# staghado/vit.cpp

Measured on AMD Instinct MI355X. Metric: images/sec ViT-B/16 224^2 bs=256 per GPU (forward, synthetic, HBM-resident inputs), higher is better.
Workload: dtype bf16; 1 GPU; vit_base_patch16_224 bf16, batch=256/GPU, 224x224x3 f32 HWC in HBM, random-init f16 file; graph=whole reference graph (every token row of every layer), global_batch=256, parallelism=single GPU

## Files before the change

include/vitx.h:

```cpp
#ifndef VITX_H
#define VITX_H

#include <stddef.h>
#include <stdint.h>

#ifdef __cplusplus
extern "C" {
#endif

typedef struct vitx_model vitx_model;
typedef struct vitx_ctx vitx_ctx;

enum vitx_status {
    VITX_OK = 0,
    VITX_ERR_IO = 1,
    VITX_ERR_FORMAT = 2,
    VITX_ERR_ARG = 3,
    VITX_ERR_HIP = 4,
    VITX_ERR_UNSUPPORTED = 5,
    VITX_ERR_NOMEM = 6
};

enum vitx_dtype { VITX_F16 = 0, VITX_BF16 = 1, VITX_MXFP8 = 2 };

// ... 190 lines not shown
int vitx_feat_enable(vitx_ctx *c, int flags, uint64_t layer_mask);
int vitx_feat_floats(const vitx_ctx *c);
int vitx_feat_images(const vitx_ctx *c);
int vitx_feat_read(vitx_ctx *c, float *out, size_t n_floats);
const void *vitx_feat_device(const vitx_ctx *c);
int vitx_op_features(const void *d_x, long row_stride, long img_stride, const void *d_w, const void *d_b,
                     void *d_cls, void *d_mean, void *d_tokens, long out_img_stride,
                     int n_img, int N, int D, float eps, int l2, void *stream);
int vitx_op_features_ex(const void *d_x, long row_stride, long img_stride, const void *d_w, const void *d_b,
                        void *d_cls, void *d_mean, void *d_tokens, long out_img_stride,
                        int n_img, int N, int first, int D, float eps, int l2, void *d_z, int dtype, void *stream);
int vitx_op_patch_embed_rect(int dtype, const void *d_img , const void *d_w, const void *d_bias, const void *d_pos, const void *d_cls,
                             const void *d_reg, int R, int n_img, int img_h, int img_w, int P, int Cin, int D, void *d_X);
int vitx_op_patch_embed(int dtype, const void *d_img, const void *d_w, const void *d_bias, const void *d_pos, const void *d_cls, const void *d_reg, int R,
                        void *d_X, int n_img, int S, int P, int Cin, int D, void *stream);
int vitx_op_attention_pool(const void *d_x, long row_stride, long img_stride, const void *d_ln_w, const void *d_ln_b, float eps, const void *d_u, void *d_M,
                           void *d_p , int n_img, int N, int D, int H, void *stream);

enum vitx_zs_kind { VITX_ZS_SOFTMAX = 0, VITX_ZS_SIGMOID = 1 };
int vitx_zeroshot_set(vitx_ctx *c, const float *bank , int K, int E, int kind, float scale, float bias);
int vitx_zeroshot_classes(const vitx_ctx *c);
int vitx_zeroshot_images(const vitx_ctx *c);
int vitx_zeroshot_read(vitx_ctx *c, float *probs , float *logits , size_t n_floats_each);
const void *vitx_zeroshot_device(const vitx_ctx *c);
int vitx_zeroshot_max_classes(int E);
int vitx_op_zeroshot(int dtype, const void *d_z, long z_stride, const void *d_bank ,
                     void *d_a_scratch, void *d_acc_scratch, void *d_probs, void *d_logits, int n, int K, int E, int kind, float scale, float bias, void *stream);

enum vitx_nn_source { VITX_NN_LOGITS = 0, VITX_NN_EMBED = 1 };
int vitx_nn_width(const vitx_ctx *c, int source);
// ... 98 lines not shown
```

vit.cpp_amd/binding.py:

```python
from __future__ import annotations

import ctypes as C
import os
import subprocess
from typing import List, Optional, Tuple

import numpy as np

from .ggml_file import (ACT_TANH as ACT_GELU_TANH, ACT_ERF as ACT_GELU_ERF, ACT_QUICK as ACT_QUICK_GELU,
                        ZS_SOFTMAX, ZS_SIGMOID, POOL_CLS, POOL_CLS_MEAN, POOL_MAP,
                        PP_REF_BICUBIC, PP_REF_BILINEAR, PP_PIL_BILINEAR, PP_PIL_BICUBIC, PP_STRETCH, PP_SHORTEST_EDGE)

_HERE = os.path.dirname(os.path.abspath(__file__))
LIB_PATH = os.environ.get("VITX_LIB") or os.path.join(_HERE, "libvitx.so")

F16, BF16, MXFP8 = 0, 1, 2
LN_TEST_KEY = 0x7e570000
BICUBIC, BILINEAR = 0, 1
EPI_BIAS, EPI_BIAS_GELU, EPI_BIAS_RESID, EPI_BIAS_F32, EPI_PATCH, EPI_BIAS_HILO = 0, 1, 2, 3, 4, 5
EPI_BIAS_GELU_ERF, EPI_BIAS_QGELU = 6, 7
ERR_IO, ERR_FORMAT, ERR_ARG, ERR_HIP, ERR_UNSUPPORTED, ERR_NOMEM = 1, 2, 3, 4, 5, 6
GEMM_AUTO, GEMM_PP, GEMM_AUTO_SPLIT = 0, 1, 2
ATTN_AUTO, ATTN_SINGLE, ATTN_FLOW, ATTN_PERSIST, ATTN_STREAM = 0, 1, 3, 4, 5
ATTN_ROLLOUT = 1
# ... 21 lines not shown
    "vitx_model_num_registers", "vitx_model_head_pool", "vitx_ctx_registers", "vitx_op_features_ex", "vitx_op_patch_embed",
    "vitx_model_activation", "vitx_model_has_pre_norm", "vitx_op_layernorm_f32",
    "vitx_model_preproc", "vitx_model_has_preproc", "vitx_preproc_at_size", "vitx_preprocess_ex", "vitx_preprocess_ex_device", "vitx_preprocess_ex_device_supports",
    "vitx_model_num_prefix", "vitx_model_pool_query", "vitx_op_attention_pool",
    "vitx_zeroshot_set", "vitx_zeroshot_classes", "vitx_zeroshot_images", "vitx_zeroshot_read", "vitx_zeroshot_device", "vitx_zeroshot_max_classes", "vitx_op_zeroshot",
    "vitx_nn_width", "vitx_nn_set", "vitx_nn_rows", "vitx_nn_k", "vitx_nn_labels", "vitx_nn_images", "vitx_nn_read", "vitx_nn_device", "vitx_nn_scratch_bytes",
    "vitx_op_nn_select", "vitx_op_nn_finish", "vitx_op_nn_state_bytes", "vitx_op_nn",
    "vitx_dense_set", "vitx_dense_classes", "vitx_dense_shape", "vitx_dense_images", "vitx_dense_read", "vitx_dense_device", "vitx_dense_scratch_bytes",
    "vitx_op_dense_labels", "vitx_dense_labels_host", "vitx_op_dense",
    "vitx_depth_set", "vitx_depth_bins", "vitx_depth_shape", "vitx_depth_images", "vitx_depth_read", "vitx_depth_device", "vitx_depth_scratch_bytes",
    "vitx_op_depth_fine", "vitx_op_depth_resize", "vitx_depth_host", "vitx_op_depth", "vitx_op_depth_rows",
    "vitx_model_kind", "vitx_model_text_info", "vitx_model_text_zs", "vitx_text_create", "vitx_text_free", "vitx_text_embed", "vitx_text_embed_device", "vitx_text_shares_weights", "vitx_text_check_ids",
    "vitx_op_text_embed", "vitx_op_text_pool", "vitx_op_attention_text", "vitx_op_attention_generic",
    "vitx_model_rope", "vitx_model_rope_table", "vitx_op_rope",
    "vitx_model_glu", "vitx_op_swiglu",
    "vitx_ctx_create_rect", "vitx_ctx_img_shape", "vitx_ctx_grid", "vitx_op_patch_embed_rect",
    "vitx_rect_shape", "vitx_preprocess_rect", "vitx_preprocess_rect_device", "vitx_preprocess_rect_device_supports",
    "vitx_pack_create", "vitx_pack_free", "vitx_pack_shares_weights", "vitx_pack_check", "vitx_pack_distinct_grids", "vitx_pack_forward", "vitx_pack_forward_device",
    "vitx_pack_feat_enable", "vitx_pack_feat_read", "vitx_pack_scratch_bytes", "vitx_pack_launches", "vitx_op_attention_packed", "vitx_op_attention_packed_tables", "vitx_op_rope_packed",
]


class HParams(C.Structure):
    _fields_ = [("hidden_size", C.c_int32), ("num_hidden_layers", C.c_int32), ("num_attention_heads", C.c_int32), ("num_classes", C.c_int32),
                ("patch_size", C.c_int32), ("img_size", C.c_int32), ("ftype", C.c_int32), ("eps", C.c_float)]


class CtxOptions(C.Structure):
    _fields_ = [("struct_size", C.c_int32), ("streams", C.c_int32), ("graph", C.c_int32), ("quant_on_host", C.c_int32), ("q4_fused_rows", C.c_int32),
                ("split_first", C.c_int32), ("no_ln_fusion", C.c_int32), ("ln_test", C.c_int32), ("f16_fast_attention", C.c_int32), ("last_layer_all_rows", C.c_int32),
                ("img_size", C.c_int32), ("pos_interp", C.c_int32)]
# ... 215 lines not shown
            L.vitx_op_attention_text.argtypes = [ip, vp, vp, ip, ip, ip, ip, ip, vp]
            L.vitx_op_attention_generic.argtypes = [ip, vp, vp, ip, ip, ip, ip, vp]
        if hasattr(L, "vitx_op_rope"):
            L.vitx_model_rope.argtypes = [vp, C.POINTER(ip), C.POINTER(C.c_float)]
            L.vitx_model_rope_table.argtypes = [vp, ip, ip, C.POINTER(C.c_float), C.POINTER(C.c_float)]
            L.vitx_op_rope.argtypes = [ip, vp, C.c_long, vp, vp, ip, ip, ip, ip, ip, vp]
        if hasattr(L, "vitx_op_swiglu"):
            L.vitx_model_glu.argtypes = [vp, C.POINTER(ip), C.POINTER(ip)]
            L.vitx_op_swiglu.argtypes = [ip, vp, C.c_long, vp, C.c_long, C.c_long, ip, vp]
        if hasattr(L, "vitx_ctx_create_rect"):
            pp = C.POINTER(Preproc)
            L.vitx_ctx_create_rect.argtypes = [vp, ip, ip, ip, C.POINTER(CtxOptions), ip, ip, C.POINTER(vp)]
            L.vitx_ctx_img_shape.argtypes = [vp, C.POINTER(ip), C.POINTER(ip)]
            L.vitx_ctx_grid.argtypes = [vp, C.POINTER(ip), C.POINTER(ip)]
            L.vitx_op_patch_embed_rect.argtypes = [ip, vp, vp, vp, vp, vp, vp, ip, ip, ip, ip, ip, ip, ip, vp]
            L.vitx_rect_shape.argtypes = [ip, ip, ip, ip, ip, C.POINTER(ip), C.POINTER(ip)]
            L.vitx_preprocess_rect.argtypes = [pp, C.POINTER(C.c_uint8), ip, ip, ip, ip, C.POINTER(C.c_float)]
            L.vitx_preprocess_rect_device.argtypes = [pp, vp, ip, ip, ip, ip, ip, vp, vp]
            L.vitx_preprocess_rect_device_supports.argtypes = [pp, ip, ip, ip, ip]
        if hasattr(L, "vitx_pack_create"):
            i32p, fp = C.POINTER(C.c_int32), C.POINTER(C.c_float)
            L.vitx_pack_create.argtypes = [vp, ip, ip, ip, ip, C.POINTER(PackOptions), C.POINTER(vp)]
            L.vitx_pack_free.argtypes = [vp]
            L.vitx_pack_shares_weights.argtypes = [vp]
            L.vitx_pack_check.argtypes = [vp, i32p, ip, ip, ip, i32p]
            L.vitx_pack_distinct_grids.argtypes = [vp, i32p, ip]
            L.vitx_pack_forward.argtypes = [vp, fp, i32p, ip, fp, fp]
            L.vitx_pack_forward_device.argtypes = [vp, vp, i32p, ip, vp, vp, vp]
            L.vitx_pack_feat_enable.argtypes = [vp, ip]
            L.vitx_pack_feat_read.argtypes = [vp, fp, fp]
# ... 872 lines not shown
                   n_img: int, N: int, first: int, D: int, eps: float = 1e-6, l2: bool = False, d_z: int = 0, dtype: int = F16, stream: int = 0) -> None:
    check(lib().vitx_op_features_ex(d_x, row_stride, img_stride, d_w, d_b, d_cls or None, d_mean or None, d_tokens or None, out_img_stride,
                                    n_img, N, first, D, eps, int(l2), d_z or None, dtype, stream or None), "vitx_op_features_ex")


def op_patch_embed(dtype: int, d_img: int, d_w: int, d_bias: int, d_pos: int, d_cls: int, d_reg: int, R: int, d_X: int, n_img: int, S: int, P: int,
                   Cin: int, D: int, stream: int = 0) -> None:
    check(lib().vitx_op_patch_embed(dtype, d_img, d_w, d_bias, d_pos, d_cls or None, d_reg or None, R, d_X, n_img, S, P, Cin, D, stream or None), "vitx_op_patch_embed")


def op_patch_embed_rect(dtype: int, d_img: int, d_w: int, d_bias: int, d_pos: int, d_cls: int, d_reg: int, R: int, d_X: int, n_img: int, img_h: int, img_w: int,
                        P: int, Cin: int, D: int) -> None:
    check(lib().vitx_op_patch_embed_rect(dtype, d_img, d_w, d_bias, d_pos, d_cls or None, d_reg or None, R, n_img, img_h, img_w, P, Cin, D, d_X), "vitx_op_patch_embed_rect")


def op_attention_pool(d_x: int, row_stride: int, img_stride: int, d_ln_w: int, d_ln_b: int, eps: float, d_u: int, d_M: int, d_p: int,
                      n_img: int, N: int, D: int, H: int, stream: int = 0) -> None:
    check(lib().vitx_op_attention_pool(d_x, row_stride, img_stride, d_ln_w, d_ln_b, eps, d_u, d_M, d_p or None, n_img, N, D, H, stream or None), "vitx_op_attention_pool")


def op_rope(dtype: int, d_qkv: int, d_cos: int, d_sin: int, n_img: int, N: int, prefix: int, D: int, H: int, lo_off: int = 0, stream: int = 0) -> None:
    check(lib().vitx_op_rope(dtype, d_qkv, lo_off, d_cos, d_sin, n_img, N, prefix, D, H, stream), "vitx_op_rope")


def op_swiglu(dtype: int, d_in: int, ld_in: int, d_out: int, ld_out: int, rows: int, F: int, stream: int = 0) -> None:
    check(lib().vitx_op_swiglu(dtype, d_in, ld_in, d_out, ld_out, rows, F, stream or None), "vitx_op_swiglu")


def op_text_embed(table_f16: bool, d_tok: int, d_pos: int, d_ids: int, d_x: int, n: int, T: int, D: int, stream: int = 0) -> None:
    check(lib().vitx_op_text_embed(1 if table_f16 else 0, d_tok, d_pos, d_ids, d_x, n, T, D, stream), "vitx_op_text_embed")
# ... 204 lines not shown
```

vit.cpp_amd/csrc/kernels.h:

```cpp
#pragma once
#include <hip/hip_runtime.h>
#include <stdint.h>

#include <type_traits>

#include "../../include/vitx.h"

namespace vitx {

enum { DT_F16 = 0, DT_BF16 = 1 };

enum {
    EPI_BIAS = 0,
    EPI_BIAS_GELU = 1,
    EPI_BIAS_RESID = 2,
    EPI_BIAS_F32 = 3,
    EPI_PATCH = 4,
    EPI_BIAS_HILO = 5,
    EPI_BIAS_GELU_ERF = 6,
    EPI_BIAS_QGELU = 7
};
constexpr int EPI_COUNT = 8;
constexpr __host__ __device__ bool epi_is_act(int epi) { return epi == EPI_BIAS_GELU || epi == EPI_BIAS_GELU_ERF || epi == EPI_BIAS_QGELU; }
constexpr __host__ __device__ int epi_act(int epi) { return epi == EPI_BIAS_GELU_ERF ? 1 : epi == EPI_BIAS_QGELU ? 2 : 0; }
// ... 61 lines not shown
    int attn_grid = 0;
};
const Tuning *tuning_for_device(int device);

hipError_t launch_gemm(const Tuning &t, int dtype, int epi, const GemmArgs &a, hipStream_t stream);
bool gemm_ln_fusable(const Tuning &t, const GemmArgs &a);
bool gemm_fix_capable(const Tuning &t, const GemmArgs &a);
int gemm_ln_grid(int n_cu, int M, int N);
hipError_t launch_layernorm_fixup(int dtype, const float *x, const float *w, const float *b, void *y, int M, int D, float eps, const unsigned *todo, unsigned epoch, hipStream_t stream);
int gemm_ring_cfg(const Tuning &t, const GemmArgs &a);
int gemm_tile_m();
int gemm_tile_n();

hipError_t launch_patch_embed(int dtype, const float *img, const void *w_perm, const float *bias, const float *pos, const float *cls, const float *reg, int n_reg,
                              float *X, int n_img, int img_h, int img_w, int P, int Cin, int D, int n_pad, int k_pad, hipStream_t stream);
void patch_embed_permute_k(const uint16_t *w, uint16_t *w_perm, int N, int Cin, int P, int k_pad);
hipError_t launch_layernorm(int dtype, const float *x, long ldx, const float *w, const float *b, void *y, long ldy, int M, int D, float eps, hipStream_t stream, int group = 1, long gstride = 0);
hipError_t launch_layernorm_f32(const float *x, const float *w, const float *b, float *y, int M, int D, float eps, hipStream_t stream);
hipError_t launch_attention(const Tuning &t, int dtype, const void *qkv, void *out, int n_img, int N, int D, int H, hipStream_t stream);
hipError_t launch_attention_stream(int dtype, bool precise, const void *qkv, void *out, int n_img, int N, int D, int H, long lo_off, hipStream_t stream);
bool attention_stream_supports(int n_img, int N, int D, int H);
hipError_t launch_split_hilo(int dtype, const float *x, void *hi, void *lo, size_t n, hipStream_t stream);
hipError_t launch_attention_cls(int dtype, const void *qkv, long lo_off, void *out, const float *x, float *xc, int n_img, int N, int D, int H, hipStream_t stream);
bool attention_cls_supports(int N, int D, int H);
constexpr int kAttnMeanMaxTokens = 1024;
bool attention_map_supports(int N, int D, int H);
bool attention_mean_supports(int N, int D, int H);
hipError_t launch_attention_cls_map(int dtype, const void *qkv, long lo_off, float *out, long img_stride, int n_img, int N, int D, int H, hipStream_t stream);
hipError_t launch_attention_head_mean(int dtype, const void *qkv, long lo_off, float *out, int n_img, int N, int D, int H, bool half_identity, hipStream_t stream);
hipError_t launch_rollout_step(float *a, const float *r, int n_img, int N, hipStream_t stream);
// ... 98 lines not shown
```

vit.cpp_amd/csrc/ops.cpp:

```cpp
#include <cmath>
#include <initializer_list>

#include "context.h"
#include "preproc_resample.h"
#include "dense_resample.h"

static int op_rc(const char *name, hipError_t e, int invalid = VITX_ERR_HIP) {
    if (e == hipSuccess) return VITX_OK;
    set_error("%s: %s", name, hipGetErrorString(e));
    return e == hipErrorInvalidValue ? invalid : VITX_ERR_HIP;
}
static bool lo_plane_ok(const char *name, int dtype, long lo_off, long hi_elems) {
    if (!lo_off || (dtype == VITX_F16 && lo_off >= hi_elems && lo_off % 8 == 0)) return true;
    set_error("%s: a lo plane needs VITX_F16 and lo_off %ld a multiple of 8 elements, at least n_img * N * 3 * D = %ld", name, lo_off, hi_elems);
    return false;
}

extern "C" {

int vitx_op_layernorm(int dtype, const void *x, const void *w, const void *b, void *y, int M, int D, float eps, void *stream) {
    if (!x || !w || !b || !y || M <= 0) return VITX_ERR_ARG;
    return op_rc("vitx_op_layernorm", launch_layernorm(dtype, (const float *)x, D, (const float *)w, (const float *)b, y, D, M, D, eps, (hipStream_t)stream), VITX_ERR_UNSUPPORTED);
}
int vitx_op_layernorm_f32(const void *x, const void *w, const void *b, void *y, int M, int D, float eps, void *stream) {
// ... 229 lines not shown
        if ((uintptr_t)p % 16) { set_error("%s: pointers must be 16-byte aligned", name); return VITX_ERR_ARG; }
    if (row_stride % 4 || img_stride % 4 || out_img_stride % 4) { set_error("%s: strides must be multiples of 4 floats", name); return VITX_ERR_ARG; }
    if (!layernorm_supports(D)) { set_error("%s: hidden size %d has no LayerNorm instantiation", name, D); return VITX_ERR_UNSUPPORTED; }
    return op_rc(name, launch_features((const float *)d_x, row_stride, img_stride, (const float *)d_w, (const float *)d_b, (float *)d_cls, (float *)d_mean, (float *)d_tokens,
                                       out_img_stride, n_img, N, D, eps, l2 != 0, (hipStream_t)stream, first, d_z, dtype));
}
int vitx_op_features(const void *d_x, long row_stride, long img_stride, const void *d_w, const void *d_b, void *d_cls, void *d_mean, void *d_tokens, long out_img_stride,
                     int n_img, int N, int D, float eps, int l2, void *stream) {
    return op_features("vitx_op_features", false, d_x, row_stride, img_stride, d_w, d_b, d_cls, d_mean, d_tokens, out_img_stride, n_img, N, 1, D, eps, l2, nullptr, VITX_F16, stream);
}
int vitx_op_features_ex(const void *d_x, long row_stride, long img_stride, const void *d_w, const void *d_b, void *d_cls, void *d_mean, void *d_tokens, long out_img_stride,
                        int n_img, int N, int first, int D, float eps, int l2, void *d_z, int dtype, void *stream) {
    return op_features("vitx_op_features_ex", true, d_x, row_stride, img_stride, d_w, d_b, d_cls, d_mean, d_tokens, out_img_stride, n_img, N, first, D, eps, l2, d_z, dtype, stream);
}
static int op_patch_embed(const char *name, int dtype, const void *d_img, const void *d_w, const void *d_bias, const void *d_pos, const void *d_cls, const void *d_reg, int R, void *d_X,
                          int n_img, int img_h, int img_w, int P, int Cin, int D, void *stream) {
    if (!d_img || !d_w || !d_bias || !d_pos || (!d_cls && R != 0) || !d_X || R < 0 || (R > 0 && !d_reg) || n_img <= 0 || img_h <= 0 || img_w <= 0 || P <= 0 || img_h % P || img_w % P ||
        Cin <= 0 || D <= 0 || D % 4 || (dtype != VITX_F16 && dtype != VITX_BF16)) { set_error("%s: invalid argument", name); return VITX_ERR_ARG; }
    if (!tuning_for_device(-1)) { set_error("%s: kernel bring-up failed", name); return VITX_ERR_HIP; }
    const int K = Cin * P * P, k_pad = round_up(K, 64), n_pad = round_up(D, gemm_tile_n());
    std::vector<float> wf((size_t)D * K);
    HIP_TRY(hipMemcpy(wf.data(), d_w, wf.size() * 4, hipMemcpyDeviceToHost));
    const std::vector<uint16_t> hp = operand_matrix_host(dtype, wf.data(), nullptr, D, K, n_pad, k_pad, P, Cin);
    void *w_perm = nullptr; float *bias = nullptr;
    HIP_TRY(hipMalloc(&w_perm, hp.size() * 2));
    const DevMem w_own(w_perm);
    if (hipMalloc((void **)&bias, (size_t)n_pad * 4) != hipSuccess) return VITX_ERR_NOMEM;
    const DevMem bias_own(bias);
    hipStream_t st = (hipStream_t)stream;
    hipError_t e = hipMemcpy(w_perm, hp.data(), hp.size() * 2, hipMemcpyHostToDevice);
    if (e == hipSuccess) e = hipMemset(bias, 0, (size_t)n_pad * 4);
    if (e == hipSuccess) e = hipMemcpy(bias, d_bias, (size_t)D * 4, hipMemcpyDeviceToDevice);
    if (e == hipSuccess) e = launch_patch_embed(dtype, (const float *)d_img, w_perm, bias, (const float *)d_pos, (const float *)d_cls, (const float *)d_reg, R,
                                                (float *)d_X, n_img, img_h, img_w, P, Cin, D, n_pad, k_pad, st);
    if (e == hipSuccess) e = hipStreamSynchronize(st);
    return op_rc(name, e, VITX_ERR_UNSUPPORTED);
}
int vitx_op_patch_embed(int dtype, const void *d_img, const void *d_w, const void *d_bias, const void *d_pos, const void *d_cls, const void *d_reg, int R, void *d_X,
                        int n_img, int S, int P, int Cin, int D, void *stream) {
    return op_patch_embed("vitx_op_patch_embed", dtype, d_img, d_w, d_bias, d_pos, d_cls, d_reg, R, d_X, n_img, S, S, P, Cin, D, stream);
}
int vitx_op_patch_embed_rect(int dtype, const void *d_img, const void *d_w, const void *d_bias, const void *d_pos, const void *d_cls, const void *d_reg, int R,
                             int n_img, int img_h, int img_w, int P, int Cin, int D, void *d_X) {
    return op_patch_embed("vitx_op_patch_embed_rect", dtype, d_img, d_w, d_bias, d_pos, d_cls, d_reg, R, d_X, n_img, img_h, img_w, P, Cin, D, nullptr);
}
int vitx_op_attention_pool(const void *d_x, long row_stride, long img_stride, const void *d_ln_w, const void *d_ln_b, float eps, const void *d_u, void *d_M, void *d_p,
                           int n_img, int N, int D, int H, void *stream) {
    if (!d_x || !d_ln_w || !d_ln_b || !d_u || !d_M || n_img <= 0 || N <= 0 || D <= 0 || H <= 0 || H > kPoolMaxHeads) { set_error("vitx_op_attention_pool: invalid argument (1 <= H <= %d)", kPoolMaxHeads); return VITX_ERR_ARG; }
    for (const void *p : {d_x, d_ln_w, d_ln_b, d_u, (const void *)d_M, (const void *)d_p})
        if ((uintptr_t)p % 16) { set_error("vitx_op_attention_pool: pointers must be 16-byte aligned"); return VITX_ERR_ARG; }
    if (row_stride % 4 || img_stride % 4) { set_error("vitx_op_attention_pool: strides must be multiples of 4 floats"); return VITX_ERR_ARG; }
    if (!layernorm_supports(D)) { set_error("vitx_op_attention_pool: hidden size %d has no LayerNorm instantiation", D); return VITX_ERR_UNSUPPORTED; }
    return op_rc("vitx_op_attention_pool", launch_attention_pool((const float *)d_x, row_stride, img_stride, (const float *)d_ln_w, (const float *)d_ln_b, eps, (const float *)d_u,
                                                                 (float *)d_M, nullptr, DT_F16, (float *)d_p, n_img, N, D, H, (hipStream_t)stream), VITX_ERR_UNSUPPORTED);
}
int vitx_op_attention_map(int dtype, const void *d_qkv, long lo_off, void *d_cls, void *d_mean, int n_img, int N, int D, int H, void *stream) {
    if (!d_qkv || (!d_cls && !d_mean) || n_img <= 0 || N <= 0 || D <= 0 || H <= 0 || (dtype != VITX_F16 && dtype != VITX_BF16)) { set_error("vitx_op_attention_map: invalid argument"); return VITX_ERR_ARG; }
    if (!lo_plane_ok("vitx_op_attention_map", dtype, lo_off, (long)n_img * N * 3 * D)) return VITX_ERR_ARG;
    if (!attention_map_supports(N, D, H)) { set_error("vitx_op_attention_map: head_dim must be a multiple of 8 up to 128 (D %d, H %d)", D, H); return VITX_ERR_UNSUPPORTED; }
// ... 235 lines not shown
```

vit.cpp_amd/csrc/patch_embed.hip:

```cpp
#include "device_common.h"
#include "kernels.h"
#include "epilogue16.h"

namespace vitx {

namespace pe {
constexpr int BM = 128, BN = 128, BK = 64;
constexpr int TILE = BM * BK * 2, STAGE = 2 * TILE, LDS_BYTES = 2 * STAGE;
}

template <typename T>
__global__ __launch_bounds__(256) void patch_embed_kernel(GemmArgs g, const float *__restrict__ img, const float *__restrict__ cls, const float *__restrict__ reg, int IH, int IW , int P, int Cin, int gw ) {
    using namespace pe;
    extern __shared__ __attribute__((aligned(16))) char smem[];
    typedef typename Elem<T>::v8 v8;
    const int tid = threadIdx.x, lane = tid & 63;
    const int wave = __builtin_amdgcn_readfirstlane(tid >> 6);
    const int l15 = lane & 15, g4 = lane >> 4;

    const int nwg = gridDim.x, bid = blockIdx.x;
    const int q8 = nwg >> 3, r8 = nwg & 7, xcd = bid & 7;
    const int tile = (xcd < r8 ? xcd * (q8 + 1) : r8 * (q8 + 1) + (xcd - r8) * q8) + (bid >> 3);
    const int ntn = g.N_pad / BN;
    const int m0 = (tile / ntn) * BM, n0 = (tile % ntn) * BN;

    const T *W = (const T *)g.W;
    int woff[4];
#pragma unroll
    for (int i = 0; i < 4; ++i) { int row, slot; swz_inv(i * 256 + tid, row, slot); woff[i] = (n0 + row) * g.ldw + slot * 8; }
    auto stage_w = [&](int buf, int k0) {
        char *base = smem + buf * STAGE + TILE + wave * 1024;
#pragma unroll
        for (int i = 0; i < 4; ++i) __builtin_amdgcn_global_load_lds(GPTR(W + woff[i] + k0), LPTR(base + i * 4096), 16, 0, 0);
    };
    const int a_row = tid >> 1, a_h = tid & 1;
    const int K = Cin * P * P, PC = P * Cin, tpi = g.tpi;
    const int m = m0 + a_row;
    const bool row_ok = m < g.M_real;
    const float *prow;
    {
        const int b = m / tpi, t = m - b * tpi, py = t / gw, px = t - py * gw;
        prow = img + (((size_t)b * IH + (size_t)py * P) * IW + (size_t)px * P) * Cin;
    }
    const bool fast = (PC & 15) == 0;
    f32x4 areg[2][4];
    auto load_a = [&](int kt) {
#pragma unroll
        for (int q = 0; q < 2; ++q) {
            const int k0 = kt * BK + (a_h * 2 + q) * 16;
            if (fast) {
                const int ky = k0 / PC, r0 = k0 - ky * PC;
                const f32x4 *src = (const f32x4 *)(prow + (size_t)ky * IW * Cin + r0);
                const bool ok = row_ok && k0 < K;
#pragma unroll
                for (int e = 0; e < 4; ++e) areg[q][e] = ok ? src[e] : f32x4{0.0f, 0.0f, 0.0f, 0.0f};
            } else {
#pragma unroll
                for (int e = 0; e < 16; ++e) {
                    const int k = k0 + e, ky = k / PC, r = k - ky * PC;
                    areg[q][e >> 2][e & 3] = (row_ok && k < K) ? prow[(size_t)ky * IW * Cin + r] : 0.0f;
                }
            }
        }
    };
    auto write_a = [&](int buf) {
        char *at = smem + buf * STAGE;
#pragma unroll
        for (int q = 0; q < 2; ++q)
#pragma unroll
            for (int hh = 0; hh < 2; ++hh) {
                const f32x4 lo = areg[q][2 * hh], hi = areg[q][2 * hh + 1];
                const typename Pair<T>::v2 p0 = round_pair<T>(lo[0], lo[1]), p1 = round_pair<T>(lo[2], lo[3]), p2 = round_pair<T>(hi[0], hi[1]), p3 = round_pair<T>(hi[2], hi[3]);
                *(v8 *)(at + swz_byte(a_row, (a_h * 2 + q) * 2 + hh)) = v8{p0[0], p0[1], p1[0], p1[1], p2[0], p2[1], p3[0], p3[1]};
            }
    };

    const int wm = wave >> 1, wn = wave & 1;
    f32x4 acc[4][4];
#pragma unroll
    for (int t = 0; t < 4; ++t)
#pragma unroll
        for (int u = 0; u < 4; ++u) acc[t][u] = f32x4{0.0f, 0.0f, 0.0f, 0.0f};
    int a_rd[4][2], w_rd[4][2];
#pragma unroll
    for (int t = 0; t < 4; ++t)
#pragma unroll
        for (int k2 = 0; k2 < 2; ++k2) {
            a_rd[t][k2] = swz_byte(wm * 64 + t * 16 + l15, k2 * 4 + g4);
            w_rd[t][k2] = TILE + swz_byte(wn * 64 + t * 16 + l15, k2 * 4 + g4);
        }

    const int nk = g.K / BK;
    stage_w(0, 0);
    load_a(0); write_a(0);
    asm volatile("s_waitcnt vmcnt(0)" ::: "memory");
    __syncthreads();
    for (int kt = 0; kt < nk; ++kt) {
        const int cur = kt & 1;
        if (kt + 1 < nk) { stage_w(cur ^ 1, (kt + 1) * BK); load_a(kt + 1); }
        const char *sb = smem + cur * STAGE;
#pragma unroll
        for (int k2 = 0; k2 < 2; ++k2) {
            v8 af[4], wf[4];
#pragma unroll
            for (int t = 0; t < 4; ++t) { af[t] = *(const v8 *)(sb + a_rd[t][k2]); wf[t] = *(const v8 *)(sb + w_rd[t][k2]); }
#pragma unroll
            for (int t = 0; t < 4; ++t)
#pragma unroll
                for (int u = 0; u < 4; ++u) acc[t][u] = Elem<T>::mfma16(wf[u], af[t], acc[t][u]);
        }
        if (kt + 1 < nk) write_a(cur ^ 1);
        asm volatile("s_waitcnt vmcnt(0)" ::: "memory");
        __syncthreads();
    }
    const bool full = (m0 + BM <= g.M_real) && (n0 + BN <= g.N);
    const int row0 = m0 + wm * 64 + l15, col0 = n0 + wn * 64 + 4 * g4;
    if (full) epilogue16<T, EPI_PATCH, 4, 4, true>(g, acc, row0, col0);
    else epilogue16<T, EPI_PATCH, 4, 4, false>(g, acc, row0, col0);
    if (g.prefix == 0) return;
#pragma unroll
    for (int t = 0; t < 4; ++t) {
        const int row = row0 + t * 16;
        if (row >= g.M_real || row % tpi) continue;
        float *o = (float *)g.out + ((size_t)row + (size_t)(row / tpi) * g.prefix) * g.ldo;
#pragma unroll
        for (int u = 0; u < 4; ++u)
#pragma unroll
            for (int e = 0; e < 4; ++e) { const int c = col0 + u * 16 + e; if (c < g.N) o[c] = cls[c] + g.pos[c]; }
// ... 5 lines not shown
#pragma unroll
                for (int e = 0; e < 4; ++e) { const int c = col0 + u * 16 + e; if (c < g.N) orow[c] = src[c]; }
        }
    }
}

void patch_embed_permute_k(const uint16_t *w, uint16_t *w_perm, int N, int Cin, int P, int k_pad) {
    const int K = Cin * P * P;
    for (int n = 0; n < N; ++n)
        for (int c = 0; c < Cin; ++c)
            for (int y = 0; y < P; ++y)
                for (int x = 0; x < P; ++x) w_perm[(size_t)n * k_pad + (y * P + x) * Cin + c] = w[(size_t)n * k_pad + c * P * P + y * P + x];
    (void)K;
}

hipError_t prepare_patch_embed() {
    hipError_t e = hipFuncSetAttribute((const void *)patch_embed_kernel<_Float16>, hipFuncAttributeMaxDynamicSharedMemorySize, pe::LDS_BYTES);
    if (e != hipSuccess) return e;
    return hipFuncSetAttribute((const void *)patch_embed_kernel<__bf16>, hipFuncAttributeMaxDynamicSharedMemorySize, pe::LDS_BYTES);
}

hipError_t launch_patch_embed(int dtype, const float *img, const void *w_perm, const float *bias, const float *pos, const float *cls, const float *reg, int n_reg,
                              float *X, int n_img, int img_h, int img_w, int P, int Cin, int D, int n_pad, int k_pad, hipStream_t stream) {
    if (n_img <= 0 || P <= 0 || img_h <= 0 || img_w <= 0 || img_h % P || img_w % P || n_pad % pe::BN || k_pad % pe::BK || k_pad < Cin * P * P || D % 4 || n_reg < 0 || (n_reg > 0 && (!reg || !cls))) return hipErrorInvalidValue;
    const int gh = img_h / P, gw = img_w / P, tpi = gh * gw;
    if ((long)n_img * tpi > 0x7fffff00l) return hipErrorInvalidValue;
    GemmArgs g{};
    g.W = w_perm; g.bias = bias; g.out = X; g.pos = pos;
    g.M_real = n_img * tpi; g.M = (g.M_real + pe::BM - 1) / pe::BM * pe::BM; g.N = D; g.N_pad = n_pad; g.K = k_pad; g.ldw = k_pad; g.ldo = D; g.tpi = tpi; g.prefix = cls ? 1 + n_reg : 0;
    const int grid = (g.M / pe::BM) * (n_pad / pe::BN);
    if (dtype == DT_F16) hipLaunchKernelGGL(patch_embed_kernel<_Float16>, dim3(grid), dim3(256), pe::LDS_BYTES, stream, g, img, cls, reg, img_h, img_w, P, Cin, gw);
    else hipLaunchKernelGGL(patch_embed_kernel<__bf16>, dim3(grid), dim3(256), pe::LDS_BYTES, stream, g, img, cls, reg, img_h, img_w, P, Cin, gw);
    return hipGetLastError();
}

}
```

Measured before the change: 27010 images/s.

## Add wide-tile triple-buffered patch-embed kernel with direct LDS DMA for weights

Rewrites the patch-embedding GEMM kernel so the weight operand uses three LDS buffers filled by inline global_load_lds DMA. Image loads are issued two k-steps ahead with partial vmcnt waits in place of a full drain every iteration. It also adds a 256-column tile variant with 512 threads, chosen automatically when the grid still covers all CUs, and compile-time FAST/slow im2col paths using 32-bit offsets. The goal is to hide global-load latency and improve weight reuse in the patch embed, at the cost of more template instances, more registers and tighter offset-range limits.

```diff
diff --git a/include/vitx.h b/include/vitx.h
--- a/include/vitx.h
+++ b/include/vitx.h
@@ -228,6 +228,8 @@
                              const void *d_reg, int R, int n_img, int img_h, int img_w, int P, int Cin, int D, void *d_X);
 int vitx_op_patch_embed(int dtype, const void *d_img, const void *d_w, const void *d_bias, const void *d_pos, const void *d_cls, const void *d_reg, int R,
                         void *d_X, int n_img, int S, int P, int Cin, int D, void *stream);
+int vitx_op_patch_embed_ex(int dtype, const void *d_img, const void *d_w, const void *d_bias, const void *d_pos, const void *d_cls, const void *d_reg, int R,
+                           int n_img, int img_h, int img_w, int P, int Cin, int D, void *d_X, int width);
 int vitx_op_attention_pool(const void *d_x, long row_stride, long img_stride, const void *d_ln_w, const void *d_ln_b, float eps, const void *d_u, void *d_M,
                            void *d_p , int n_img, int N, int D, int H, void *stream);
 
diff --git a/vit.cpp_amd/binding.py b/vit.cpp_amd/binding.py
--- a/vit.cpp_amd/binding.py
+++ b/vit.cpp_amd/binding.py
@@ -59,7 +59,7 @@
     "vitx_op_text_embed", "vitx_op_text_pool", "vitx_op_attention_text", "vitx_op_attention_generic",
     "vitx_model_rope", "vitx_model_rope_table", "vitx_op_rope",
     "vitx_model_glu", "vitx_op_swiglu",
-    "vitx_ctx_create_rect", "vitx_ctx_img_shape", "vitx_ctx_grid", "vitx_op_patch_embed_rect",
+    "vitx_ctx_create_rect", "vitx_ctx_img_shape", "vitx_ctx_grid", "vitx_op_patch_embed_rect", "vitx_op_patch_embed_ex",
     "vitx_rect_shape", "vitx_preprocess_rect", "vitx_preprocess_rect_device", "vitx_preprocess_rect_device_supports",
     "vitx_pack_create", "vitx_pack_free", "vitx_pack_shares_weights", "vitx_pack_check", "vitx_pack_distinct_grids", "vitx_pack_forward", "vitx_pack_forward_device",
     "vitx_pack_feat_enable", "vitx_pack_feat_read", "vitx_pack_scratch_bytes", "vitx_pack_launches", "vitx_op_attention_packed", "vitx_op_attention_packed_tables", "vitx_op_rope_packed",
@@ -305,6 +305,7 @@
             L.vitx_ctx_img_shape.argtypes = [vp, C.POINTER(ip), C.POINTER(ip)]
             L.vitx_ctx_grid.argtypes = [vp, C.POINTER(ip), C.POINTER(ip)]
             L.vitx_op_patch_embed_rect.argtypes = [ip, vp, vp, vp, vp, vp, vp, ip, ip, ip, ip, ip, ip, ip, vp]
+            L.vitx_op_patch_embed_ex.argtypes = [ip, vp, vp, vp, vp, vp, vp, ip, ip, ip, ip, ip, ip, ip, vp, ip]
             L.vitx_rect_shape.argtypes = [ip, ip, ip, ip, ip, C.POINTER(ip), C.POINTER(ip)]
             L.vitx_preprocess_rect.argtypes = [pp, C.POINTER(C.c_uint8), ip, ip, ip, ip, C.POINTER(C.c_float)]
             L.vitx_preprocess_rect_device.argtypes = [pp, vp, ip, ip, ip, ip, ip, vp, vp]
@@ -1207,6 +1208,11 @@
     check(lib().vitx_op_patch_embed_rect(dtype, d_img, d_w, d_bias, d_pos, d_cls or None, d_reg or None, R, n_img, img_h, img_w, P, Cin, D, d_X), "vitx_op_patch_embed_rect")
 
 
+def op_patch_embed_ex(dtype: int, d_img: int, d_w: int, d_bias: int, d_pos: int, d_cls: int, d_reg: int, R: int, d_X: int, n_img: int, img_h: int, img_w: int,
+                      P: int, Cin: int, D: int, width: int = 0) -> None:
+    check(lib().vitx_op_patch_embed_ex(dtype, d_img, d_w, d_bias, d_pos, d_cls or None, d_reg or None, R, n_img, img_h, img_w, P, Cin, D, d_X, width), "vitx_op_patch_embed_ex")
+
+
 def op_attention_pool(d_x: int, row_stride: int, img_stride: int, d_ln_w: int, d_ln_b: int, eps: float, d_u: int, d_M: int, d_p: int,
                       n_img: int, N: int, D: int, H: int, stream: int = 0) -> None:
     check(lib().vitx_op_attention_pool(d_x, row_stride, img_stride, d_ln_w, d_ln_b, eps, d_u, d_M, d_p or None, n_img, N, D, H, stream or None), "vitx_op_attention_pool")
diff --git a/vit.cpp_amd/csrc/kernels.h b/vit.cpp_amd/csrc/kernels.h
--- a/vit.cpp_amd/csrc/kernels.h
+++ b/vit.cpp_amd/csrc/kernels.h
@@ -99,6 +99,9 @@
 
 hipError_t launch_patch_embed(int dtype, const float *img, const void *w_perm, const float *bias, const float *pos, const float *cls, const float *reg, int n_reg,
                               float *X, int n_img, int img_h, int img_w, int P, int Cin, int D, int n_pad, int k_pad, hipStream_t stream);
+int patch_embed_width(const Tuning &t, int M_pad, int n_pad);
+hipError_t launch_patch_embed_width(int width, int dtype, const float *img, const void *w_perm, const float *bias, const float *pos, const float *cls, const float *reg, int n_reg,
+                                    float *X, int n_img, int img_h, int img_w, int P, int Cin, int D, int n_pad, int k_pad, hipStream_t stream);
 void patch_embed_permute_k(const uint16_t *w, uint16_t *w_perm, int N, int Cin, int P, int k_pad);
 hipError_t launch_layernorm(int dtype, const float *x, long ldx, const float *w, const float *b, void *y, long ldy, int M, int D, float eps, hipStream_t stream, int group = 1, long gstride = 0);
 hipError_t launch_layernorm_f32(const float *x, const float *w, const float *b, float *y, int M, int D, float eps, hipStream_t stream);
diff --git a/vit.cpp_amd/csrc/ops.cpp b/vit.cpp_amd/csrc/ops.cpp
--- a/vit.cpp_amd/csrc/ops.cpp
+++ b/vit.cpp_amd/csrc/ops.cpp
@@ -267,11 +267,12 @@
     return op_features("vitx_op_features_ex", true, d_x, row_stride, img_stride, d_w, d_b, d_cls, d_mean, d_tokens, out_img_stride, n_img, N, first, D, eps, l2, d_z, dtype, stream);
 }
 static int op_patch_embed(const char *name, int dtype, const void *d_img, const void *d_w, const void *d_bias, const void *d_pos, const void *d_cls, const void *d_reg, int R, void *d_X,
-                          int n_img, int img_h, int img_w, int P, int Cin, int D, void *stream) {
+                          int n_img, int img_h, int img_w, int P, int Cin, int D, void *stream, int width = 0) {
     if (!d_img || !d_w || !d_bias || !d_pos || (!d_cls && R != 0) || !d_X || R < 0 || (R > 0 && !d_reg) || n_img <= 0 || img_h <= 0 || img_w <= 0 || P <= 0 || img_h % P || img_w % P ||
-        Cin <= 0 || D <= 0 || D % 4 || (dtype != VITX_F16 && dtype != VITX_BF16)) { set_error("%s: invalid argument", name); return VITX_ERR_ARG; }
+        Cin <= 0 || D <= 0 || D % 4 || (dtype != VITX_F16 && dtype != VITX_BF16) || (width != 0 && width != 128 && width != 256)) { set_error("%s: invalid argument", name); return VITX_ERR_ARG; }
     if (!tuning_for_device(-1)) { set_error("%s: kernel bring-up failed", name); return VITX_ERR_HIP; }
     const int K = Cin * P * P, k_pad = round_up(K, 64), n_pad = round_up(D, gemm_tile_n());
+    if (width == 256 && n_pad % 256) { set_error("%s: the 256-column build needs the padded hidden size (%d) to be a multiple of 256", name, n_pad); return VITX_ERR_UNSUPPORTED; }
     std::vector<float> wf((size_t)D * K);
     HIP_TRY(hipMemcpy(wf.data(), d_w, wf.size() * 4, hipMemcpyDeviceToHost));
     const std::vector<uint16_t> hp = operand_matrix_host(dtype, wf.data(), nullptr, D, K, n_pad, k_pad, P, Cin);
@@ -284,8 +285,8 @@
     hipError_t e = hipMemcpy(w_perm, hp.data(), hp.size() * 2, hipMemcpyHostToDevice);
     if (e == hipSuccess) e = hipMemset(bias, 0, (size_t)n_pad * 4);
     if (e == hipSuccess) e = hipMemcpy(bias, d_bias, (size_t)D * 4, hipMemcpyDeviceToDevice);
-    if (e == hipSuccess) e = launch_patch_embed(dtype, (const float *)d_img, w_perm, bias, (const float *)d_pos, (const float *)d_cls, (const float *)d_reg, R,
-                                                (float *)d_X, n_img, img_h, img_w, P, Cin, D, n_pad, k_pad, st);
+    if (e == hipSuccess) e = launch_patch_embed_width(width, dtype, (const float *)d_img, w_perm, bias, (const float *)d_pos, (const float *)d_cls, (const float *)d_reg, R,
+                                                      (float *)d_X, n_img, img_h, img_w, P, Cin, D, n_pad, k_pad, st);
     if (e == hipSuccess) e = hipStreamSynchronize(st);
     return op_rc(name, e, VITX_ERR_UNSUPPORTED);
 }
@@ -296,6 +297,10 @@
 int vitx_op_patch_embed_rect(int dtype, const void *d_img, const void *d_w, const void *d_bias, const void *d_pos, const void *d_cls, const void *d_reg, int R,
                              int n_img, int img_h, int img_w, int P, int Cin, int D, void *d_X) {
     return op_patch_embed("vitx_op_patch_embed_rect", dtype, d_img, d_w, d_bias, d_pos, d_cls, d_reg, R, d_X, n_img, img_h, img_w, P, Cin, D, nullptr);
+}
+int vitx_op_patch_embed_ex(int dtype, const void *d_img, const void *d_w, const void *d_bias, const void *d_pos, const void *d_cls, const void *d_reg, int R,
+                           int n_img, int img_h, int img_w, int P, int Cin, int D, void *d_X, int width) {
+    return op_patch_embed("vitx_op_patch_embed_ex", dtype, d_img, d_w, d_bias, d_pos, d_cls, d_reg, R, d_X, n_img, img_h, img_w, P, Cin, D, nullptr, width);
 }
 int vitx_op_attention_pool(const void *d_x, long row_stride, long img_stride, const void *d_ln_w, const void *d_ln_b, float eps, const void *d_u, void *d_M, void *d_p,
                            int n_img, int N, int D, int H, void *stream) {
diff --git a/vit.cpp_amd/csrc/patch_embed.hip b/vit.cpp_amd/csrc/patch_embed.hip
--- a/vit.cpp_amd/csrc/patch_embed.hip
+++ b/vit.cpp_amd/csrc/patch_embed.hip
@@ -1,3 +1,5 @@
+#include <type_traits>
+
 #include "device_common.h"
 #include "kernels.h"
 #include "epilogue16.h"
@@ -5,13 +7,35 @@
 namespace vitx {
 
 namespace pe {
-constexpr int BM = 128, BN = 128, BK = 64;
-constexpr int TILE = BM * BK * 2, STAGE = 2 * TILE, LDS_BYTES = 2 * STAGE;
-}
-
-template <typename T>
-__global__ __launch_bounds__(256) void patch_embed_kernel(GemmArgs g, const float *__restrict__ img, const float *__restrict__ cls, const float *__restrict__ reg, int IH, int IW , int P, int Cin, int gw ) {
+constexpr int BM = 128, BK = 64, BN_NARROW = 128, BN_WIDE = 256;
+constexpr int A_TILE = BM * BK * 2;
+constexpr int A_BUFS = 2, W_BUFS = 3;
+template <int BN> struct Cfg {
+    static constexpr int NT = 2 * BN;
+    static constexpr int WN = BN / 64;
+    static constexpr int W_TILE = BN * BK * 2;
+    static constexpr int LDS_BYTES = A_BUFS * A_TILE + W_BUFS * W_TILE;
+    static constexpr int NQ = 4 * BM / NT;
+    static constexpr int TPR = 4 / NQ;
+    static constexpr int W_PIECES = BN * 8 / NT;
+};
+template <int N> __device__ __forceinline__ void wait_vm_lds_barrier() {
+    asm volatile("s_waitcnt vmcnt(%0) lgkmcnt(0)\n\ts_barrier" ::"n"(N) : "memory");
+    __builtin_amdgcn_sched_barrier(0);
+}
+__device__ __forceinline__ void lds_dma16(const void *src, unsigned dst) {
+    unsigned keep;
+    asm volatile("s_mov_b32 %0, m0\n\ts_mov_b32 m0, %2\n\ts_nop 0\n\tglobal_load_lds_dwordx4 %1, off\n\ts_mov_b32 m0, %0" : "=&s"(keep) : "v"(src), "s"(dst) : "memory");
+}
+typedef std::integral_constant<int, 0> S0; typedef std::integral_constant<int, 1> S1; typedef std::integral_constant<int, 2> S2;
+}
+
+template <typename T, int BN, bool FAST>
+__global__ __launch_bounds__(pe::Cfg<BN>::NT, 512 / pe::Cfg<BN>::NT) void patch_embed_kernel(GemmArgs g, const float *__restrict__ img, const float *__restrict__ cls, const float *__restrict__ reg, int IH, int IW , int P, int Cin, int gw ) {
     using namespace pe;
+    typedef Cfg<BN> C;
+    constexpr int NT = C::NT, WN = C::WN, NQ = C::NQ, W_TILE = C::W_TILE, W_PIECES = C::W_PIECES;
+    constexpr int NA = NQ * (FAST ? 4 : 16);
     extern __shared__ __attribute__((aligned(16))) char smem[];
     typedef typename Elem<T>::v8 v8;
     const int tid = threadIdx.x, lane = tid & 63;
@@ -24,58 +48,75 @@
     const int ntn = g.N_pad / BN;
     const int m0 = (tile / ntn) * BM, n0 = (tile % ntn) * BN;
 
+    char *const smem_w = smem + A_BUFS * A_TILE;
     const T *W = (const T *)g.W;
-    int woff[4];
-#pragma unroll
-    for (int i = 0; i < 4; ++i) { int row, slot; swz_inv(i * 256 + tid, row, slot); woff[i] = (n0 + row) * g.ldw + slot * 8; }
+    int woff[W_PIECES];
+#pragma unroll
+    for (int i = 0; i < W_PIECES; ++i) { int row, slot; swz_inv(i * NT + tid, row, slot); woff[i] = (n0 + row) * g.ldw + slot * 8; }
+    const unsigned lds_w = __builtin_amdgcn_readfirstlane((unsigned)(unsigned long)LPTR(smem_w + wave * 1024));
     auto stage_w = [&](int buf, int k0) {
-        char *base = smem + buf * STAGE + TILE + wave * 1024;
-#pragma unroll
-        for (int i = 0; i < 4; ++i) __builtin_amdgcn_global_load_lds(GPTR(W + woff[i] + k0), LPTR(base + i * 4096), 16, 0, 0);
-    };
-    const int a_row = tid >> 1, a_h = tid & 1;
+#pragma unroll
+        for (int i = 0; i < W_PIECES; ++i) lds_dma16(W + woff[i] + k0, lds_w + buf * W_TILE + i * (NT * 16));
+    };
+    const int a_row = tid / C::TPR, a_h = tid % C::TPR;
     const int K = Cin * P * P, PC = P * Cin, tpi = g.tpi;
     const int m = m0 + a_row;
     const bool row_ok = m < g.M_real;
-    const float *prow;
+    const int b0 = m0 / tpi;
+    const char *const img0 = (const char *)(img + (size_t)b0 * IH * IW * Cin);
+    unsigned prow;
     {
-        const int b = m / tpi, t = m - b * tpi, py = t / gw, px = t - py * gw;
-        prow = img + (((size_t)b * IH + (size_t)py * P) * IW + (size_t)px * P) * Cin;
-    }
-    const bool fast = (PC & 15) == 0;
-    f32x4 areg[2][4];
-    auto load_a = [&](int kt) {
-#pragma unroll
-        for (int q = 0; q < 2; ++q) {
-            const int k0 = kt * BK + (a_h * 2 + q) * 16;
-            if (fast) {
-                const int ky = k0 / PC, r0 = k0 - ky * PC;
-                const f32x4 *src = (const f32x4 *)(prow + (size_t)ky * IW * Cin + r0);
-                const bool ok = row_ok && k0 < K;
-#pragma unroll
-                for (int e = 0; e < 4; ++e) areg[q][e] = ok ? src[e] : f32x4{0.0f, 0.0f, 0.0f, 0.0f};
+        const int mc = row_ok ? m : g.M_real - 1;
+        const int b = mc / tpi, t = mc - b * tpi, py = t / gw, px = t - py * gw;
+        prow = ((((unsigned)(b - b0) * IH + (unsigned)py * P) * IW + (unsigned)px * P) * Cin) * 4u;
+    }
+    const unsigned pitch = (unsigned)IW * Cin * 4u;
+    const unsigned last_off = prow + (unsigned)((K - 1) / PC) * pitch + (unsigned)((K - 1) % PC) * 4u;
+    f32x4 areg[3][NQ][4];
+    auto load_a = [&](int kt, auto S) {
+#pragma unroll
+        for (int q = 0; q < NQ; ++q) {
+            const int k0 = kt * BK + (a_h * NQ + q) * 16;
+            if constexpr (FAST) {
+                const int kc = k0 < K ? k0 : 0;
+                const int ky = kc / PC, r0 = kc - ky * PC;
+                const f32x4 *src = (const f32x4 *)(img0 + (prow + (unsigned)ky * pitch + (unsigned)r0 * 4u));
+#pragma unroll
+                for (int e = 0; e < 4; ++e) areg[S.value][q][e] = src[e];
             } else {
+                const int ky0 = k0 / PC;
+                int r = k0 - ky0 * PC;
+                unsigned off = prow + (unsigned)ky0 * pitch + (unsigned)r * 4u;
+                const unsigned wrap = pitch - (unsigned)PC * 4u;
 #pragma unroll
                 for (int e = 0; e < 16; ++e) {
-                    const int k = k0 + e, ky = k / PC, r = k - ky * PC;
-                    areg[q][e >> 2][e & 3] = (row_ok && k < K) ? prow[(size_t)ky * IW * Cin + r] : 0.0f;
+                    areg[S.value][q][e >> 2][e & 3] = *(const float *)(img0 + min(off, last_off));
+                    ++r; off += 4u;
+                    if (r == PC) { r = 0; off += wrap; }
                 }
             }
         }
     };
-    auto write_a = [&](int buf) {
-        char *at = smem + buf * STAGE;
-#pragma unroll
-        for (int q = 0; q < 2; ++q)
+    auto write_a = [&](int kt, auto S) {
+        char *at = smem + (kt & 1) * A_TILE;
+#pragma unroll
+        for (int q = 0; q < NQ; ++q) {
+            const int k0 = kt * BK + (a_h * NQ + q) * 16;
+            f32x4 v[4];
+#pragma unroll
+            for (int e = 0; e < 4; ++e)
+#pragma unroll
+                for (int c = 0; c < 4; ++c) v[e][c] = (row_ok && k0 + e * 4 + c < K) ? areg[S.value][q][e][c] : 0.0f;
 #pragma unroll
             for (int hh = 0; hh < 2; ++hh) {
-                const f32x4 lo = areg[q][2 * hh], hi = areg[q][2 * hh + 1];
+                const f32x4 lo = v[2 * hh], hi = v[2 * hh + 1];
                 const typename Pair<T>::v2 p0 = round_pair<T>(lo[0], lo[1]), p1 = round_pair<T>(lo[2], lo[3]), p2 = round_pair<T>(hi[0], hi[1]), p3 = round_pair<T>(hi[2], hi[3]);
-                *(v8 *)(at + swz_byte(a_row, (a_h * 2 + q) * 2 + hh)) = v8{p0[0], p0[1], p1[0], p1[1], p2[0], p2[1], p3[0], p3[1]};
+                *(v8 *)(at + swz_byte(a_row, (a_h * NQ + q) * 2 + hh)) = v8{p0[0], p0[1], p1[0], p1[1], p2[0], p2[1], p3[0], p3[1]};
             }
-    };
-
-    const int wm = wave >> 1, wn = wave & 1;
+        }
+    };
+
+    const int wm = wave / WN, wn = wave % WN;
     f32x4 acc[4][4];
 #pragma unroll
     for (int t = 0; t < 4; ++t)
@@ -87,31 +128,57 @@
 #pragma unroll
         for (int k2 = 0; k2 < 2; ++k2) {
             a_rd[t][k2] = swz_byte(wm * 64 + t * 16 + l15, k2 * 4 + g4);
-            w_rd[t][k2] = TILE + swz_byte(wn * 64 + t * 16 + l15, k2 * 4 + g4);
+            w_rd[t][k2] = swz_byte(wn * 64 + t * 16 + l15, k2 * 4 + g4);
         }
 
     const int nk = g.K / BK;
-    stage_w(0, 0);
-    load_a(0); write_a(0);
-    asm volatile("s_waitcnt vmcnt(0)" ::: "memory");
-    __syncthreads();
-    for (int kt = 0; kt < nk; ++kt) {
-        const int cur = kt & 1;
-        if (kt + 1 < nk) { stage_w(cur ^ 1, (kt + 1) * BK); load_a(kt + 1); }
-        const char *sb = smem + cur * STAGE;
+    auto multiply = [&](int kt, int wslot) {
+        const char *sa = smem + (kt & 1) * A_TILE, *sw = smem_w + wslot * W_TILE;
 #pragma unroll
         for (int k2 = 0; k2 < 2; ++k2) {
             v8 af[4], wf[4];
 #pragma unroll
-            for (int t = 0; t < 4; ++t) { af[t] = *(const v8 *)(sb + a_rd[t][k2]); wf[t] = *(const v8 *)(sb + w_rd[t][k2]); }
+            for (int t = 0; t < 4; ++t) { af[t] = *(const v8 *)(sa + a_rd[t][k2]); wf[t] = *(const v8 *)(sw + w_rd[t][k2]); }
 #pragma unroll
             for (int t = 0; t < 4; ++t)
 #pragma unroll
                 for (int u = 0; u < 4; ++u) acc[t][u] = Elem<T>::mfma16(wf[u], af[t], acc[t][u]);
-        }
-        if (kt + 1 < nk) write_a(cur ^ 1);
-        asm volatile("s_waitcnt vmcnt(0)" ::: "memory");
-        __syncthreads();
+            if (k2 == 0) __builtin_amdgcn_sched_barrier(0);
+        }
+    };
+    auto step = [&](int kt, auto S) {
+        typedef std::integral_constant<int, (S.value + 1) % 3> SN;
+        typedef std::integral_constant<int, (S.value + 2) % 3> SNN;
+        stage_w(SNN::value, (kt + 2) * BK); load_a(kt + 2, SNN());
+        __builtin_amdgcn_sched_barrier(0);
+        multiply(kt, S.value);
+        write_a(kt + 1, SN());
+        wait_vm_lds_barrier<W_PIECES + NA>();
+    };
+    auto last_steps = [&](int kt, auto S) {
+        typedef std::integral_constant<int, (S.value + 1) % 3> SN;
+        typedef std::integral_constant<int, (S.value + 2) % 3> SNN;
+        const bool more2 = kt + 2 < nk;
+        if (more2) { stage_w(SNN::value, (kt + 2) * BK); load_a(kt + 2, SNN()); }
+        multiply(kt, S.value);
+        if (kt + 1 < nk) write_a(kt + 1, SN());
+        if (more2) wait_vm_lds_barrier<W_PIECES + NA>(); else wait_vm_lds_barrier<0>();
+    };
+    int kt = 0;
+    stage_w(0, 0); load_a(0, S0());
+    if (nk > 1) {
+        stage_w(1, BK); load_a(1, S1());
+        write_a(0, S0());
+        wait_vm_lds_barrier<W_PIECES + NA>();
+        for (; kt + 4 < nk; kt += 3) { step(kt, S0()); step(kt + 1, S1()); step(kt + 2, S2()); }
+    } else {
+        write_a(0, S0());
+        wait_vm_lds_barrier<0>();
+    }
+    for (; kt < nk; kt += 3) {
+        last_steps(kt, S0());
+        if (kt + 1 < nk) last_steps(kt + 1, S1());
+        if (kt + 2 < nk) last_steps(kt + 2, S2());
     }
     const bool full = (m0 + BM <= g.M_real) && (n0 + BN <= g.N);
     const int row0 = m0 + wm * 64 + l15, col0 = n0 + wn * 64 + 4 * g4;
@@ -147,24 +214,63 @@
     (void)K;
 }
 
+template <typename T, int BN, bool FAST>
+static hipError_t patch_embed_instance(bool prepare, const GemmArgs &g, const float *img, const float *cls, const float *reg, int img_h, int img_w, int P, int Cin, int gw, hipStream_t stream) {
+    typedef pe::Cfg<BN> C;
+    if (prepare) return hipFuncSetAttribute((const void *)patch_embed_kernel<T, BN, FAST>, hipFuncAttributeMaxDynamicSharedMemorySize, C::LDS_BYTES);
+    hipLaunchKernelGGL((patch_embed_kernel<T, BN, FAST>), dim3((g.M / pe::BM) * (g.N_pad / BN)), dim3(C::NT), C::LDS_BYTES, stream, g, img, cls, reg, img_h, img_w, P, Cin, gw);
+    return hipGetLastError();
+}
+static hipError_t patch_embed_dispatch(bool prepare, int dtype, int bn, bool fast, const GemmArgs &g, const float *img, const float *cls, const float *reg, int img_h, int img_w, int P, int Cin, int gw, hipStream_t stream) {
+#define PE_CASE(T, BN, FAST) return patch_embed_instance<T, BN, FAST>(prepare, g, img, cls, reg, img_h, img_w, P, Cin, gw, stream)
+    if (dtype == DT_F16) {
+        if (bn == pe::BN_WIDE) { if (fast) PE_CASE(_Float16, pe::BN_WIDE, true); PE_CASE(_Float16, pe::BN_WIDE, false); }
+        if (fast) PE_CASE(_Float16, pe::BN_NARROW, true);
+        PE_CASE(_Float16, pe::BN_NARROW, false);
+    }
+    if (bn == pe::BN_WIDE) { if (fast) PE_CASE(__bf16, pe::BN_WIDE, true); PE_CASE(__bf16, pe::BN_WIDE, false); }
+    if (fast) PE_CASE(__bf16, pe::BN_NARROW, true);
+    PE_CASE(__bf16, pe::BN_NARROW, false);
+#undef PE_CASE
+}
+
 hipError_t prepare_patch_embed() {
-    hipError_t e = hipFuncSetAttribute((const void *)patch_embed_kernel<_Float16>, hipFuncAttributeMaxDynamicSharedMemorySize, pe::LDS_BYTES);
-    if (e != hipSuccess) return e;
-    return hipFuncSetAttribute((const void *)patch_embed_kernel<__bf16>, hipFuncAttributeMaxDynamicSharedMemorySize, pe::LDS_BYTES);
-}
-
-hipError_t launch_patch_embed(int dtype, const float *img, const void *w_perm, const float *bias, const float *pos, const float *cls, const float *reg, int n_reg,
-                              float *X, int n_img, int img_h, int img_w, int P, int Cin, int D, int n_pad, int k_pad, hipStream_t stream) {
-    if (n_img <= 0 || P <= 0 || img_h <= 0 || img_w <= 0 || img_h % P || img_w % P || n_pad % pe::BN || k_pad % pe::BK || k_pad < Cin * P * P || D % 4 || n_reg < 0 || (n_reg > 0 && (!reg || !cls))) return hipErrorInvalidValue;
+    GemmArgs none{};
+    for (int dt = 0; dt < 2; ++dt)
+        for (int bn : {pe::BN_NARROW, pe::BN_WIDE})
+            for (int fast = 0; fast < 2; ++fast) {
+                const hipError_t e = patch_embed_dispatch(true, dt == 0 ? (int)DT_F16 : (int)DT_BF16, bn, fast != 0, none, nullptr, nullptr, nullptr, 0, 0, 0, 0, 0, nullptr);
+                if (e != hipSuccess) return e;
+            }
+    return hipSuccess;
+}
+
+int patch_embed_width(const Tuning &t, int M_pad, int n_pad) {
+    if (n_pad % pe::BN_WIDE) return pe::BN_NARROW;
+    return (long)(M_pad / pe::BM) * (n_pad / pe::BN_WIDE) >= t.n_cu ? pe::BN_WIDE : pe::BN_NARROW;
+}
+
+hipError_t launch_patch_embed_width(int width, int dtype, const float *img, const void *w_perm, const float *bias, const float *pos, const float *cls, const float *reg, int n_reg,
+                                    float *X, int n_img, int img_h, int img_w, int P, int Cin, int D, int n_pad, int k_pad, hipStream_t stream) {
+    if (n_img <= 0 || P <= 0 || Cin <= 0 || img_h <= 0 || img_w <= 0 || img_h % P || img_w % P || n_pad % pe::BN_NARROW || D > n_pad || k_pad % pe::BK || k_pad < Cin * P * P || D % 4 || n_reg < 0 || (n_reg > 0 && (!reg || !cls))) return hipErrorInvalidValue;
+    if ((dtype != DT_F16 && dtype != DT_BF16) || (width != 0 && width != pe::BN_NARROW && width != pe::BN_WIDE) || (width == pe::BN_WIDE && n_pad % pe::BN_WIDE)) return hipErrorInvalidValue;
     const int gh = img_h / P, gw = img_w / P, tpi = gh * gw;
     if ((long)n_img * tpi > 0x7fffff00l) return hipErrorInvalidValue;
+    if ((128l / tpi + 2) * img_h * img_w * Cin * 4 > 0xf0000000l) return hipErrorInvalidValue;
     GemmArgs g{};
     g.W = w_perm; g.bias = bias; g.out = X; g.pos = pos;
     g.M_real = n_img * tpi; g.M = (g.M_real + pe::BM - 1) / pe::BM * pe::BM; g.N = D; g.N_pad = n_pad; g.K = k_pad; g.ldw = k_pad; g.ldo = D; g.tpi = tpi; g.prefix = cls ? 1 + n_reg : 0;
-    const int grid = (g.M / pe::BM) * (n_pad / pe::BN);
-    if (dtype == DT_F16) hipLaunchKernelGGL(patch_embed_kernel<_Float16>, dim3(grid), dim3(256), pe::LDS_BYTES, stream, g, img, cls, reg, img_h, img_w, P, Cin, gw);
-    else hipLaunchKernelGGL(patch_embed_kernel<__bf16>, dim3(grid), dim3(256), pe::LDS_BYTES, stream, g, img, cls, reg, img_h, img_w, P, Cin, gw);
-    return hipGetLastError();
-}
-
-}
+    if (width == 0) {
+        const Tuning *t = tuning_for_device(-1);
+        if (!t) return hipErrorInvalidDevice;
+        width = patch_embed_width(*t, g.M, n_pad);
+    }
+    return patch_embed_dispatch(false, dtype, width, (P * Cin) % 16 == 0, g, img, cls, reg, img_h, img_w, P, Cin, gw, stream);
+}
+
+hipError_t launch_patch_embed(int dtype, const float *img, const void *w_perm, const float *bias, const float *pos, const float *cls, const float *reg, int n_reg,
+                              float *X, int n_img, int img_h, int img_w, int P, int Cin, int D, int n_pad, int k_pad, hipStream_t stream) {
+    return launch_patch_embed_width(0, dtype, img, w_perm, bias, pos, cls, reg, n_reg, X, n_img, img_h, img_w, P, Cin, D, n_pad, k_pad, stream);
+}
+
+}
```

Measured after the change: 27090 images/s (median of 5 runs). About the same (+0.3%).
